# zhenfeizhang/falcon-r1cs

Measured on AMD Instinct MI355X. Metric: falcon1024_verify_with_ntt_r1cs_witnesses_per_sec, higher is better.
Workload: dtype u32; 1 GPU; falcon-1024 full verify-with-ntt witness (NTT ladder + mod_q + pointwise + l2-norm), batch=65536 signatures per GPU per step (BASELINE configs[2] on every GPU); logn=10, batch_per_gpu=65536, chunk=32768, encoding=bls12-381-fr montgomery (arkworks witness_assignment bytes), seed=0x46414c434f4e31, signatures_failing_range_checks=0, ranks_seen=1, hbm_plan_bytes=166888865792, hbm_plan_limit_bytes=259200000000

## Files before the change

### falcon-r1cs_amd/csrc/frw_prepare.hip

```cpp
#include <hip/hip_runtime.h>
#include <stdint.h>
#include <algorithm>
#include "frw_device.h"
#include "frw_keccak.h"
#include "frw_layout.h"

namespace frw {

constexpr int SHAKE256_RATE = 136;
constexpr int NONCE_LEN = 40;

__device__ __forceinline__ void hash_to_point_one(int logn, const uint8_t *__restrict__ nonce, const uint8_t *__restrict__ msg, uint64_t o0,
                                         uint64_t o1, uint16_t *__restrict__ out)
{
    const int n = 1 << logn;
    const size_t total = NONCE_LEN + (size_t)(o1 >= o0 ? o1 - o0 : 0);
    uint64_t st[25];
#pragma unroll
    for (int i = 0; i < 25; i++) st[i] = 0;
    for (size_t pos = 0;; pos += SHAKE256_RATE) {
#pragma unroll
        for (int l = 0; l < SHAKE256_RATE / 8; l++) {
            uint64_t w = 0;
#pragma unroll
            for (int b = 0; b < 8; b++) {
                const size_t p = pos + (size_t)(l * 8 + b);
                uint32_t byte = 0;
                if (p < NONCE_LEN) byte = nonce[p];
                else if (p < total) byte = msg[p - NONCE_LEN];
                else if (p == total) byte = 0x1F;
                w |= (uint64_t)byte << (8 * b);
            }
            st[l] ^= w;
        }
        const bool last = total < pos + SHAKE256_RATE;
        if (last) st[16] ^= 0x8000000000000000ull;
        keccak_f1600(st);
        if (last) break;
    }
    int cnt = 0;
    while (cnt < n) {
#pragma unroll
        for (int w = 0; w < SHAKE256_RATE / 2; w++) {
            const uint64_t lane = st[w / 4];
            const int sh = (w % 4) * 16;
            const uint32_t v = (uint32_t)((lane >> sh) & 0xff) << 8 | (uint32_t)((lane >> (sh + 8)) & 0xff);
            if (v < 5 * Q && cnt < n) out[cnt++] = (uint16_t)(v % Q);
        }
        if (cnt < n) keccak_f1600(st);
    }
}

__global__ __launch_bounds__(BLOCK) void hash_to_point_kernel(int logn, size_t batch, const uint8_t *__restrict__ nonces,
                                                              const uint8_t *__restrict__ msgs,
                                                              const uint64_t *__restrict__ msg_off, uint16_t *__restrict__ hm)
{
    const size_t s = (size_t)blockIdx.x * blockDim.x + threadIdx.x;
    if (s >= batch) return;
    const uint64_t o0 = msg_off[s], o1 = msg_off[s + 1];
    hash_to_point_one(logn, nonces + s * NONCE_LEN, msgs + o0, o0, o1, hm + (s << logn));
}

__device__ __forceinline__ uint32_t public_key_coeff(const uint8_t *__restrict__ p, int k)
{
    const int bit = 14 * k, off = bit & 7;
    const uint8_t *q = p + 1 + (bit >> 3);
    uint32_t acc = (uint32_t)q[0] << 16 | (uint32_t)q[1] << 8;
    if (off + 14 > 16) acc |= q[2];
    return (acc >> (24 - 14 - off)) & 0x3fffu;
}

__global__ __launch_bounds__(BLOCK) void decode_public_keys_kernel(int logn, size_t batch, const uint8_t *__restrict__ pk_bytes,
                                                                   uint16_t *__restrict__ pk, int32_t *__restrict__ status)
{
    const int n = 1 << logn;
    const size_t pk_len = 1 + (size_t)14 * n / 8;
    const size_t idx = (size_t)blockIdx.x * blockDim.x + threadIdx.x;
    if (idx >= batch * (size_t)n) return;
    const size_t s = idx >> logn;
    const int k = (int)(idx & (size_t)(n - 1));
    const uint8_t *p = pk_bytes + s * pk_len;
    const uint32_t c = public_key_coeff(p, k);
    pk[idx] = (uint16_t)c;
    if (c >= Q || (k == 0 && p[0] != (uint8_t)logn)) atomicMax(&status[s], ST_DECODE);
}

__device__ __forceinline__ bool decode_signature_one(int logn, const uint8_t *__restrict__ p, size_t sig_len, uint16_t *__restrict__ out,
                                            uint8_t *__restrict__ nonce_out)
{
    const int n = 1 << logn;
    bool ok = sig_len > 1 + NONCE_LEN && p[0] == (uint8_t)(0x30 + logn);
    if (ok && nonce_out)
        for (int i = 0; i < NONCE_LEN; i++) nonce_out[i] = p[1 + i];
    const uint8_t *body = p + 1 + NONCE_LEN;
    const size_t body_len = ok ? sig_len - 1 - NONCE_LEN : 0;
    size_t v = 0;
    uint32_t acc = 0;
    int acc_len = 0;
    for (int u = 0; ok && u < n; u++) {
        if (v >= body_len) { ok = false; break; }
        acc = (acc << 8) | body[v++];
        const uint32_t b = acc >> acc_len;
        const uint32_t sign = b & 128u;
        uint32_t m = b & 127u;
        for (;;) {
            if (acc_len == 0) {
                if (v >= body_len) { ok = false; break; }
                acc = (acc << 8) | body[v++];
                acc_len = 8;
            }
            acc_len--;
            if ((acc >> acc_len) & 1u) break;
            m += 128;
            if (m > 2047) { ok = false; break; }
        }
        if (sign && m == 0) ok = false;
        if (ok) out[u] = (uint16_t)(sign ? Q - m : m);
    }
    if (ok && (acc & ((1u << acc_len) - 1u))) ok = false;
    for (; ok && v < body_len; v++)
        if (body[v]) ok = false;
    return ok;
}

__global__ __launch_bounds__(BLOCK) void decode_signatures_kernel(int logn, size_t batch, const uint8_t *__restrict__ sig_bytes,
                                                                  size_t sig_len, uint16_t *__restrict__ sig,
                                                                  uint8_t *__restrict__ nonce_out, int32_t *__restrict__ status)
{
    const size_t s = (size_t)blockIdx.x * blockDim.x + threadIdx.x;
    if (s >= batch) return;
    const bool ok = decode_signature_one(logn, sig_bytes + s * sig_len, sig_len, sig + (s << logn),
                                         nonce_out ? nonce_out + s * NONCE_LEN : nullptr);
    status[s] = ok ? ST_OK : ST_DECODE;
}

__global__ __launch_bounds__(BLOCK) void agg_hash_to_point_kernel(int logn, size_t count, const uint32_t *__restrict__ stmt,
                                                                  const uint8_t *__restrict__ nonces, const uint8_t *__restrict__ msgs,
                                                                  const uint64_t *__restrict__ msg_off, uint16_t *__restrict__ hm)
{
    const size_t k = (size_t)blockIdx.x * blockDim.x + threadIdx.x;
    if (k >= count) return;
    const size_t s = stmt[k];
    const uint64_t o0 = msg_off[s], o1 = msg_off[s + 1];
    hash_to_point_one(logn, nonces + aggregate_route(logn - 9, k, s).nonce_off, msgs + o0, o0, o1, hm + (k << logn));
}

__global__ __launch_bounds__(BLOCK) void agg_decode_public_keys_kernel(int logn, size_t count, const uint32_t *__restrict__ stmt,
                                                                       const uint8_t *__restrict__ pk_bytes, uint16_t *__restrict__ pk,
                                                                       int32_t *__restrict__ status)
{
    const int n = 1 << logn;
    const size_t idx = (size_t)blockIdx.x * blockDim.x + threadIdx.x;
    if (idx >= count * (size_t)n) return;
    const size_t k = idx >> logn;
    const int j = (int)(idx & (size_t)(n - 1));
    const uint8_t *p = pk_bytes + aggregate_route(logn - 9, k, stmt[k]).pk_off;
    const uint32_t c = public_key_coeff(p, j);
    pk[idx] = (uint16_t)c;
    if (c >= Q || (j == 0 && p[0] != (uint8_t)logn)) atomicMax(&status[k], ST_DECODE);
}

__global__ __launch_bounds__(BLOCK) void agg_decode_signatures_kernel(int logn, size_t count, const uint32_t *__restrict__ stmt,
                                                                      const uint8_t *__restrict__ sig_bytes, uint16_t *__restrict__ sig,
                                                                      uint8_t *__restrict__ nonces, int32_t *__restrict__ status)
{
    const size_t k = (size_t)blockIdx.x * blockDim.x + threadIdx.x;
    if (k >= count) return;
    const AggRoute r = aggregate_route(logn - 9, k, stmt[k]);
    const uint8_t *p = sig_bytes + r.sig_off;
    for (int i = 0; i < NONCE_LEN; i++) nonces[r.nonce_off + i] = p[1 + i];
    status[k] = decode_signature_one(logn, p, aggregate_sig_len(logn - 9), sig + (k << logn), nullptr) ? ST_OK : ST_DECODE;
}

struct AggVerdicts { const uint32_t *stmt[2]; const int32_t *status[2]; const uint64_t *norm[2]; uint32_t count[2]; };
__global__ __launch_bounds__(BLOCK) void agg_scatter_verdicts_kernel(AggVerdicts v, int32_t *__restrict__ status, uint64_t *__restrict__ norm)
{
    size_t k = (size_t)blockIdx.x * blockDim.x + threadIdx.x;
    int g = 0;
    if (k >= v.count[0]) { k -= v.count[0]; g = 1; }
    if (k >= v.count[g]) return;
    const size_t s = v.stmt[g][k];
    status[s] = v.status[g][k];
    if (norm) norm[s] = v.norm[g][k];
}

__global__ __launch_bounds__(BLOCK) void agg_count_refused_kernel(size_t count, const int32_t *__restrict__ status, uint32_t *__restrict__ refused)
{
    __shared__ uint32_t wave_count[WAVES];
    uint32_t mine = 0;
    for (size_t s = threadIdx.x; s < count; s += BLOCK) mine += status[s] != ST_OK;
#pragma unroll
    for (int off = WAVE / 2; off > 0; off >>= 1) mine += __shfl_xor(mine, off, WAVE);
    if ((threadIdx.x & (WAVE - 1)) == 0) wave_count[threadIdx.x / WAVE] = mine;
    __syncthreads();
    if (threadIdx.x == 0) {
        uint32_t total = 0;
#pragma unroll
        for (int w = 0; w < WAVES; w++) total += wave_count[w];
        refused[0] = total;
    }
}


__device__ inline uint32_t pok_block_rank(bool flag, uint32_t &total)
{
    __shared__ uint32_t wave_count[WAVES];
    const uint64_t mask = __ballot(flag);
    const int lane = threadIdx.x & (WAVE - 1), wave = threadIdx.x / WAVE;
    if (lane == 0) wave_count[wave] = (uint32_t)__popcll(mask);
    __syncthreads();
    uint32_t before = 0;
    total = 0;
#pragma unroll
    for (int w = 0; w < WAVES; w++) {
        if (w < wave) before += wave_count[w];
        total += wave_count[w];
    }
    return before + (uint32_t)__popcll(mask & (((uint64_t)1 << lane) - 1));
}

__global__ __launch_bounds__(BLOCK) void pok_scan_count_kernel(size_t batch, const int32_t *__restrict__ status,
                                                               uint32_t *__restrict__ block_sums)
{
    const size_t s = (size_t)blockIdx.x * BLOCK + threadIdx.x;
    uint32_t total;
    (void)pok_block_rank(s < batch && status[s] == ST_OK, total);
    if (threadIdx.x == 0) block_sums[blockIdx.x] = total;
}

__global__ __launch_bounds__(BLOCK) void pok_scan_offsets_kernel(size_t num_blocks, uint32_t *__restrict__ block_sums,
                                                                 uint32_t *__restrict__ count)
{
    __shared__ uint32_t wave_sum[WAVES];
    const int lane = threadIdx.x & (WAVE - 1), wave = threadIdx.x / WAVE;
    uint32_t carry = 0;
    for (size_t base = 0; base < num_blocks; base += BLOCK) {
        const size_t i = base + threadIdx.x;
        const uint32_t v = i < num_blocks ? block_sums[i] : 0;
        uint32_t incl = v;
#pragma unroll
        for (int d = 1; d < WAVE; d <<= 1) {
            const uint32_t up = __shfl_up(incl, d, WAVE);
            if (lane >= d) incl += up;
        }
        if (lane == WAVE - 1) wave_sum[wave] = incl;
        __syncthreads();
        uint32_t before = 0, tile = 0;
#pragma unroll
        for (int w = 0; w < WAVES; w++) {
            if (w < wave) before += wave_sum[w];
            tile += wave_sum[w];
        }
        if (i < num_blocks) block_sums[i] = carry + before + incl - v;
        carry += tile;
        __syncthreads();
    }
    if (threadIdx.x == 0) count[0] = carry;
}

__global__ __launch_bounds__(BLOCK) void pok_scan_write_kernel(size_t batch, const int32_t *__restrict__ status,
                                                               const uint32_t *__restrict__ block_offsets, uint32_t *__restrict__ index)
{
    const size_t s = (size_t)blockIdx.x * BLOCK + threadIdx.x;
    const bool ok = s < batch && status[s] == ST_OK;
    uint32_t total;
    const uint32_t rank = pok_block_rank(ok, total);
    if (ok) index[block_offsets[blockIdx.x] + rank] = (uint32_t)s;
}

__global__ __launch_bounds__(BLOCK) void pok_gather_rs_kernel(size_t count, const uint32_t *__restrict__ index,
                                                              const uint64_t *__restrict__ rs, uint64_t *__restrict__ dense_rs)
{
    const size_t t = (size_t)blockIdx.x * BLOCK + threadIdx.x;
    if (t >= count * 8) return;
    dense_rs[t] = rs[(size_t)index[t / 8] * 8 + (t & 7)];
}

__global__ __launch_bounds__(BLOCK) void pok_gather_inputs_kernel(int logn, const uint32_t *__restrict__ index,
                                                                  const uint16_t *__restrict__ sig, const uint16_t *__restrict__ pk,
                                                                  const uint16_t *__restrict__ hm, uint16_t *__restrict__ sig_out,
                                                                  uint16_t *__restrict__ pk_out, uint16_t *__restrict__ hm_out)
{
    const size_t j = blockIdx.x, slot = index[j];
    const uint32_t row = (2u << logn) / 16;
    for (uint32_t t = threadIdx.x; t < 3 * row; t += BLOCK) {
        const uint32_t a = t / row, v = t % row;
        const uint16_t *src = a == 0 ? sig : a == 1 ? pk : hm;
        uint16_t *dst = a == 0 ? sig_out : a == 1 ? pk_out : hm_out;
        ((uint4 *)dst)[j * row + v] = ((const uint4 *)src)[slot * row + v];
    }
}

struct PokOutputs { uint8_t *wire; uint64_t *proofs, *instance; uint32_t *unsatisfied; uint32_t wire_len, inst_words; };

__global__ __launch_bounds__(BLOCK) void pok_zero_refused_kernel(size_t batch, const int32_t *__restrict__ status, PokOutputs out)
{
    for (size_t s = blockIdx.x; s < batch; s += gridDim.x) {
        if (status[s] == ST_OK) continue;
        for (uint32_t t = threadIdx.x; t < out.wire_len; t += BLOCK) out.wire[s * out.wire_len + t] = 0;
        if (out.proofs && threadIdx.x < 48) out.proofs[s * 48 + threadIdx.x] = 0;
        if (out.instance)
            for (uint32_t t = threadIdx.x; t < out.inst_words; t += BLOCK) out.instance[s * out.inst_words + t] = 0;
        if (out.unsatisfied && threadIdx.x == 0) out.unsatisfied[s] = 0;
    }
}

__global__ __launch_bounds__(BLOCK) void pok_scatter_kernel(const uint32_t *__restrict__ index, const uint8_t *__restrict__ wire,
                                                            const uint64_t *__restrict__ proofs, const uint64_t *__restrict__ instance,
                                                            const uint32_t *__restrict__ unsatisfied, PokOutputs out)
{
    const size_t j = blockIdx.x, s = index[j];
    for (uint32_t t = threadIdx.x; t < out.wire_len; t += BLOCK) out.wire[s * out.wire_len + t] = wire[j * out.wire_len + t];
    if (out.proofs && threadIdx.x < 48) out.proofs[s * 48 + threadIdx.x] = proofs[j * 48 + threadIdx.x];
    if (out.instance)
        for (uint32_t t = threadIdx.x; t < out.inst_words; t += BLOCK) out.instance[s * out.inst_words + t] = instance[j * out.inst_words + t];
    if (out.unsatisfied && threadIdx.x == 0) out.unsatisfied[s] = unsatisfied[j];
}

hipError_t launch_pok_scan(size_t batch, const int32_t *status, uint32_t *block_sums, uint32_t *index, uint32_t *count, hipStream_t st)
{
    if (batch == 0) return hipSuccess;
    const size_t blocks = (batch + BLOCK - 1) / BLOCK;
    hipLaunchKernelGGL(pok_scan_count_kernel, dim3((unsigned)blocks), dim3(BLOCK), 0, st, batch, status, block_sums);
    hipLaunchKernelGGL(pok_scan_offsets_kernel, dim3(1), dim3(BLOCK), 0, st, blocks, block_sums, count);
    hipLaunchKernelGGL(pok_scan_write_kernel, dim3((unsigned)blocks), dim3(BLOCK), 0, st, batch, status, (const uint32_t *)block_sums, index);
    return hipGetLastError();
}

hipError_t launch_pok_gather_rs(size_t count, const uint32_t *index, const uint64_t *rs, uint64_t *dense_rs, hipStream_t st)
{
    if (count == 0) return hipSuccess;
    hipLaunchKernelGGL(pok_gather_rs_kernel, dim3((unsigned)((count * 8 + BLOCK - 1) / BLOCK)), dim3(BLOCK), 0, st, count, index, rs, dense_rs);
    return hipGetLastError();
}

hipError_t launch_pok_gather_inputs(int logn, size_t cnt, const uint32_t *index, const uint16_t *sig, const uint16_t *pk, const uint16_t *hm,
                                    uint16_t *sig_out, uint16_t *pk_out, uint16_t *hm_out, hipStream_t st)
{
    if (cnt == 0) return hipSuccess;
    hipLaunchKernelGGL(pok_gather_inputs_kernel, dim3((unsigned)cnt), dim3(BLOCK), 0, st, logn, index, sig, pk, hm, sig_out, pk_out, hm_out);
    return hipGetLastError();
}

hipError_t launch_pok_zero_refused(size_t batch, const int32_t *status, int wire_len, int inst_words, uint8_t *wire, uint64_t *proofs,
                                   uint64_t *instance, uint32_t *unsatisfied, hipStream_t st)
{
    if (batch == 0) return hipSuccess;
    const PokOutputs out = {wire, proofs, instance, unsatisfied, (uint32_t)wire_len, (uint32_t)inst_words};
    hipLaunchKernelGGL(pok_zero_refused_kernel, dim3((unsigned)std::min<size_t>(batch, 65536)), dim3(BLOCK), 0, st, batch, status, out);
    return hipGetLastError();
}

hipError_t launch_pok_scatter(size_t cnt, const uint32_t *index, int wire_len, int inst_words, const uint8_t *wire_in,
                              const uint64_t *proofs_in, const uint64_t *instance_in, const uint32_t *unsatisfied_in, uint8_t *wire,
                              uint64_t *proofs, uint64_t *instance, uint32_t *unsatisfied, hipStream_t st)
{
    if (cnt == 0) return hipSuccess;
    const PokOutputs out = {wire, proofs, instance, unsatisfied, (uint32_t)wire_len, (uint32_t)inst_words};
    hipLaunchKernelGGL(pok_scatter_kernel, dim3((unsigned)cnt), dim3(BLOCK), 0, st, index, wire_in, proofs_in, instance_in, unsatisfied_in, out);
    return hipGetLastError();
}

hipError_t launch_hash_to_point(int logn, size_t batch, const uint8_t *nonces, const uint8_t *msgs, const uint64_t *msg_off,
                                uint16_t *hm, hipStream_t st)
{
    if (batch == 0) return hipSuccess;
    hipLaunchKernelGGL(hash_to_point_kernel, dim3((unsigned)((batch + BLOCK - 1) / BLOCK)), dim3(BLOCK), 0, st, logn, batch, nonces,
                       msgs, msg_off, hm);
    return hipGetLastError();
}

hipError_t launch_decode_public_keys(int logn, size_t batch, const uint8_t *pk_bytes, uint16_t *pk, int32_t *status, hipStream_t st)
{
    if (batch == 0) return hipSuccess;
    hipError_t e = hipMemsetAsync(status, 0, batch * sizeof(int32_t), st);
    if (e != hipSuccess) return e;
    const size_t total = batch << logn;
    hipLaunchKernelGGL(decode_public_keys_kernel, dim3((unsigned)((total + BLOCK - 1) / BLOCK)), dim3(BLOCK), 0, st, logn, batch,
                       pk_bytes, pk, status);
    return hipGetLastError();
}

hipError_t launch_decode_signatures(int logn, size_t batch, const uint8_t *sig_bytes, size_t sig_len, uint16_t *sig,
                                    uint8_t *nonce_out, int32_t *status, hipStream_t st)
{
    if (batch == 0) return hipSuccess;
    hipLaunchKernelGGL(decode_signatures_kernel, dim3((unsigned)((batch + BLOCK - 1) / BLOCK)), dim3(BLOCK), 0, st, logn, batch,
                       sig_bytes, sig_len, sig, nonce_out, status);
    return hipGetLastError();
}

hipError_t launch_agg_hash_to_point(int logn, size_t count, const uint32_t *stmt, const uint8_t *nonces, const uint8_t *msgs,
                                    const uint64_t *msg_off, uint16_t *hm, hipStream_t st)
{
    if (count == 0) return hipSuccess;
    hipLaunchKernelGGL(agg_hash_to_point_kernel, dim3((unsigned)((count + BLOCK - 1) / BLOCK)), dim3(BLOCK), 0, st, logn, count, stmt, nonces,
                       msgs, msg_off, hm);
    return hipGetLastError();
}

hipError_t launch_agg_decode_public_keys(int logn, size_t count, const uint32_t *stmt, const uint8_t *pk_bytes, uint16_t *pk, int32_t *status,
                                         hipStream_t st)
{
    if (count == 0) return hipSuccess;
    hipError_t e = hipMemsetAsync(status, 0, count * sizeof(int32_t), st);
    if (e != hipSuccess) return e;
    const size_t total = count << logn;
    hipLaunchKernelGGL(agg_decode_public_keys_kernel, dim3((unsigned)((total + BLOCK - 1) / BLOCK)), dim3(BLOCK), 0, st, logn, count, stmt,
                       pk_bytes, pk, status);
    return hipGetLastError();
}

hipError_t launch_agg_decode_signatures(int logn, size_t count, const uint32_t *stmt, const uint8_t *sig_bytes, uint16_t *sig, uint8_t *nonces,
                                        int32_t *status, hipStream_t st)
{
    if (count == 0) return hipSuccess;
    hipLaunchKernelGGL(agg_decode_signatures_kernel, dim3((unsigned)((count + BLOCK - 1) / BLOCK)), dim3(BLOCK), 0, st, logn, count, stmt,
                       sig_bytes, sig, nonces, status);
    return hipGetLastError();
}

hipError_t launch_agg_verdicts(const uint32_t *const stmt[2], const int32_t *const set_status[2], const uint64_t *const set_norm[2],
                               const size_t count[2], int32_t *status, uint64_t *norm, uint32_t *refused, hipStream_t st)
{
    const size_t total = count[0] + count[1];
    if (total == 0) return hipSuccess;
    const AggVerdicts v = {{stmt[0], stmt[1]}, {set_status[0], set_status[1]}, {set_norm[0], set_norm[1]}, {(uint32_t)count[0], (uint32_t)count[1]}};
    hipLaunchKernelGGL(agg_scatter_verdicts_kernel, dim3((unsigned)((total + BLOCK - 1) / BLOCK)), dim3(BLOCK), 0, st, v, status, norm);
    hipLaunchKernelGGL(agg_count_refused_kernel, dim3(1), dim3(BLOCK), 0, st, total, (const int32_t *)status, refused);
    return hipGetLastError();
}

}
```

Before: 1.341 million signatures/s.

## Decode signatures with 16-byte vector loads and a branchless bit-stream decoder

Replaces the byte-at-a-time Falcon signature decoder with a streaming decoder that fetches 16-byte granules with prefetch-ahead, decodes coefficients via count-leading-zeros on a 64-bit bit buffer, and writes eight packed coefficients per 16-byte store. The decode kernel now launches one wave per block, and the public-key decode error flag uses a wave ballot so only one lane issues the atomic. The aim is to cut the per-byte load and store traffic and the branchy per-bit loop in the per-signature serial decode. It adds a bytewise fallback path and relies on aligned output and a correct reimplementation of the validity checks.

```diff
diff --git a/falcon-r1cs_amd/csrc/frw_prepare.hip b/falcon-r1cs_amd/csrc/frw_prepare.hip
--- a/falcon-r1cs_amd/csrc/frw_prepare.hip
+++ b/falcon-r1cs_amd/csrc/frw_prepare.hip
@@ -4,11 +4,13 @@
 #include "frw_device.h"
 #include "frw_keccak.h"
 #include "frw_layout.h"
+#include "frw_sigdecode.h"
 
 namespace frw {
 
 constexpr int SHAKE256_RATE = 136;
 constexpr int NONCE_LEN = 40;
+static_assert(SIG_Q == Q && SIG_NONCE_LEN == NONCE_LEN, "frw_sigdecode.h is the same codec");
 
 __device__ __forceinline__ void hash_to_point_one(int logn, const uint8_t *__restrict__ nonce, const uint8_t *__restrict__ msg, uint64_t o0,
                                          uint64_t o1, uint16_t *__restrict__ out)
@@ -82,50 +84,28 @@
     const uint8_t *p = pk_bytes + s * pk_len;
     const uint32_t c = public_key_coeff(p, k);
     pk[idx] = (uint16_t)c;
-    if (c >= Q || (k == 0 && p[0] != (uint8_t)logn)) atomicMax(&status[s], ST_DECODE);
-}
-
-__device__ __forceinline__ bool decode_signature_one(int logn, const uint8_t *__restrict__ p, size_t sig_len, uint16_t *__restrict__ out,
-                                            uint8_t *__restrict__ nonce_out)
-{
-    const int n = 1 << logn;
-    bool ok = sig_len > 1 + NONCE_LEN && p[0] == (uint8_t)(0x30 + logn);
-    if (ok && nonce_out)
-        for (int i = 0; i < NONCE_LEN; i++) nonce_out[i] = p[1 + i];
-    const uint8_t *body = p + 1 + NONCE_LEN;
-    const size_t body_len = ok ? sig_len - 1 - NONCE_LEN : 0;
-    size_t v = 0;
-    uint32_t acc = 0;
-    int acc_len = 0;
-    for (int u = 0; ok && u < n; u++) {
-        if (v >= body_len) { ok = false; break; }
-        acc = (acc << 8) | body[v++];
-        const uint32_t b = acc >> acc_len;
-        const uint32_t sign = b & 128u;
-        uint32_t m = b & 127u;
-        for (;;) {
-            if (acc_len == 0) {
-                if (v >= body_len) { ok = false; break; }
-                acc = (acc << 8) | body[v++];
-                acc_len = 8;
-            }
-            acc_len--;
-            if ((acc >> acc_len) & 1u) break;
-            m += 128;
-            if (m > 2047) { ok = false; break; }
-        }
-        if (sign && m == 0) ok = false;
-        if (ok) out[u] = (uint16_t)(sign ? Q - m : m);
-    }
-    if (ok && (acc & ((1u << acc_len) - 1u))) ok = false;
-    for (; ok && v < body_len; v++)
-        if (body[v]) ok = false;
-    return ok;
-}
-
-__global__ __launch_bounds__(BLOCK) void decode_signatures_kernel(int logn, size_t batch, const uint8_t *__restrict__ sig_bytes,
-                                                                  size_t sig_len, uint16_t *__restrict__ sig,
-                                                                  uint8_t *__restrict__ nonce_out, int32_t *__restrict__ status)
+    const bool bad = c >= Q || (k == 0 && p[0] != (uint8_t)logn);
+    if (__ballot(bad) != 0 && (threadIdx.x & (WAVE - 1)) == 0) atomicMax(&status[s], ST_DECODE);
+}
+
+__global__ __launch_bounds__(WAVE) void decode_signatures_kernel(int logn, size_t batch, const uint8_t *__restrict__ sig_bytes,
+                                                                 size_t sig_len, uint16_t *__restrict__ sig,
+                                                                 uint8_t *__restrict__ nonce_out, int32_t *__restrict__ status)
+{
+    const size_t s = (size_t)blockIdx.x * blockDim.x + threadIdx.x;
+    if (s >= batch) return;
+    const uint8_t *p = sig_bytes + s * sig_len;
+    const uint32_t lead = (uint32_t)((uintptr_t)p & 15);
+    const uint4 *span = (const uint4 *)(p - lead);
+    uint4 *row = (uint4 *)(sig + (s << logn));
+    const bool ok = decode_signature_wide(logn, p, lead, sig_len, nonce_out ? nonce_out + s * NONCE_LEN : nullptr,
+                                          [span](uint32_t g) { return span[g]; }, [row](uint32_t j, const uint4 &v) { row[j] = v; });
+    status[s] = ok ? ST_OK : ST_DECODE;
+}
+
+__global__ __launch_bounds__(BLOCK) void decode_signatures_bytewise_kernel(int logn, size_t batch, const uint8_t *__restrict__ sig_bytes,
+                                                                           size_t sig_len, uint16_t *__restrict__ sig,
+                                                                           uint8_t *__restrict__ nonce_out, int32_t *__restrict__ status)
 {
     const size_t s = (size_t)blockIdx.x * blockDim.x + threadIdx.x;
     if (s >= batch) return;
@@ -385,8 +365,12 @@
                                     uint8_t *nonce_out, int32_t *status, hipStream_t st)
 {
     if (batch == 0) return hipSuccess;
-    hipLaunchKernelGGL(decode_signatures_kernel, dim3((unsigned)((batch + BLOCK - 1) / BLOCK)), dim3(BLOCK), 0, st, logn, batch,
-                       sig_bytes, sig_len, sig, nonce_out, status);
+    if (((uintptr_t)sig & 15) == 0 && sig_len > 1 + NONCE_LEN && sig_len < SIG_WIDE_MAX_LEN)
+        hipLaunchKernelGGL(decode_signatures_kernel, dim3((unsigned)((batch + WAVE - 1) / WAVE)), dim3(WAVE), 0, st, logn, batch, sig_bytes,
+                           sig_len, sig, nonce_out, status);
+    else
+        hipLaunchKernelGGL(decode_signatures_bytewise_kernel, dim3((unsigned)((batch + BLOCK - 1) / BLOCK)), dim3(BLOCK), 0, st, logn, batch,
+                           sig_bytes, sig_len, sig, nonce_out, status);
     return hipGetLastError();
 }
 
diff --git a/falcon-r1cs_amd/csrc/frw_sigdecode.h b/falcon-r1cs_amd/csrc/frw_sigdecode.h
--- /dev/null
+++ b/falcon-r1cs_amd/csrc/frw_sigdecode.h
@@ -0,0 +1,150 @@
+#pragma once
+#include <hip/hip_runtime.h>
+#include <stddef.h>
+#include <stdint.h>
+
+namespace frw {
+
+constexpr uint32_t SIG_Q = 12289;
+constexpr int SIG_NONCE_LEN = 40;
+constexpr size_t SIG_WIDE_MAX_LEN = (size_t)1 << 28;
+
+__host__ __device__ __forceinline__ bool decode_signature_one(int logn, const uint8_t *__restrict__ p, size_t sig_len, uint16_t *__restrict__ out,
+                                                     uint8_t *__restrict__ nonce_out)
+{
+    const int n = 1 << logn;
+    bool ok = sig_len > 1 + SIG_NONCE_LEN && p[0] == (uint8_t)(0x30 + logn);
+    if (ok && nonce_out)
+        for (int i = 0; i < SIG_NONCE_LEN; i++) nonce_out[i] = p[1 + i];
+    const uint8_t *body = p + 1 + SIG_NONCE_LEN;
+    const size_t body_len = ok ? sig_len - 1 - SIG_NONCE_LEN : 0;
+    size_t v = 0;
+    uint32_t acc = 0;
+    int acc_len = 0;
+    for (int u = 0; ok && u < n; u++) {
+        if (v >= body_len) { ok = false; break; }
+        acc = (acc << 8) | body[v++];
+        const uint32_t b = acc >> acc_len;
+        const uint32_t sign = b & 128u;
+        uint32_t m = b & 127u;
+        for (;;) {
+            if (acc_len == 0) {
+                if (v >= body_len) { ok = false; break; }
+                acc = (acc << 8) | body[v++];
+                acc_len = 8;
+            }
+            acc_len--;
+            if ((acc >> acc_len) & 1u) break;
+            m += 128;
+            if (m > 2047) { ok = false; break; }
+        }
+        if (sign && m == 0) ok = false;
+        if (ok) out[u] = (uint16_t)(sign ? SIG_Q - m : m);
+    }
+    if (ok && (acc & ((1u << acc_len) - 1u))) ok = false;
+    for (; ok && v < body_len; v++)
+        if (body[v]) ok = false;
+    return ok;
+}
+
+template <class Store>
+struct SigStream {
+    uint64_t buf;
+    int valid;
+    uint32_t skip, rem, u, n, tail, min_unary, max_coeff, o0, o1, o2, o3;
+    Store store;
+
+    __host__ __device__ __forceinline__ SigStream(int logn, uint32_t lead, size_t sig_len, Store store_)
+        : buf(0), valid(0), skip(8 * (lead + 1 + SIG_NONCE_LEN)), rem(8 * (uint32_t)(sig_len - 1 - SIG_NONCE_LEN)), u(0), n(1u << logn), tail(0),
+          min_unary(0xffffffffu), max_coeff(0), o0(0), o1(0), o2(0), o3(0), store(store_) {}
+
+    __host__ __device__ __forceinline__ bool refused() const { return min_unary < 0x10000u || max_coeff >= SIG_Q; }
+
+    __host__ __device__ __forceinline__ void drain()
+    {
+        while (valid >= 24 && u < n) {
+            const uint32_t hi = (uint32_t)(buf >> 32);
+            const uint32_t unary = hi << 8;
+            const uint32_t k = unary ? (uint32_t)__builtin_clz(unary) : 32u;
+            const uint32_t m = ((hi >> 24) & 127u) | (k << 7);
+            const uint32_t c = (int32_t)hi < 0 ? SIG_Q - m : m;
+            min_unary = unary < min_unary ? unary : min_unary;
+            max_coeff = c > max_coeff ? c : max_coeff;
+            buf <<= 9 + k;
+            valid -= 9 + (int)k;
+            o0 = (o0 >> 16) | (o1 << 16);
+            o1 = (o1 >> 16) | (o2 << 16);
+            o2 = (o2 >> 16) | (o3 << 16);
+            o3 = (o3 >> 16) | (c << 16);
+            if ((u & 7) == 7) store(u >> 3, make_uint4(o0, o1, o2, o3));
+            u++;
+        }
+        const bool done = u == n;
+        tail |= done ? (uint32_t)(buf != 0) : 0u;
+        buf = done ? 0 : buf;
+        valid = done ? 0 : valid;
+    }
+
+    __host__ __device__ __forceinline__ void word(uint32_t le)
+    {
+        const uint32_t drop = skip < 32 ? skip : 32, bits = 32 - drop, take = bits < rem ? bits : rem;
+        uint32_t w = drop < 32 ? __builtin_bswap32(le) << drop : 0u;
+        w = take ? w & (0xffffffffu << (32 - take)) : 0u;
+        skip -= drop;
+        rem -= take;
+        const bool done = u == n;
+        tail |= done ? w : 0u;
+        buf |= (uint64_t)(done ? 0u : w) << (32 - valid);
+        valid += done ? 0 : (int)bits;
+        drain();
+    }
+
+    __host__ __device__ __forceinline__ bool granule(const uint4 &q)
+    {
+        word(q.x);
+        word(q.y);
+        word(q.z);
+        word(q.w);
+        return !refused();
+    }
+
+    __host__ __device__ __forceinline__ bool finish()
+    {
+        while (u < n) {
+            valid += 32;
+            drain();
+            if (refused()) return false;
+        }
+        return tail == 0;
+    }
+};
+
+template <class Fetch, class Store>
+__host__ __device__ __forceinline__ bool decode_signature_wide(int logn, const uint8_t *__restrict__ p, uint32_t lead, size_t sig_len,
+                                                      uint8_t *__restrict__ nonce_out, Fetch fetch, Store store)
+{
+    const uint32_t last = (uint32_t)((lead + sig_len - 1) >> 4);
+    if (p[0] != (uint8_t)(0x30 + logn)) return false;
+    if (nonce_out)
+        for (int i = 0; i < SIG_NONCE_LEN; i++) nonce_out[i] = p[1 + i];
+    const auto ahead = [&](uint32_t g) { return fetch(g < last ? g : last); };
+    uint4 q0 = ahead(0), q1 = ahead(1), q2 = ahead(2), q3 = ahead(3);
+    SigStream<Store> s(logn, lead, sig_len, store);
+    for (uint32_t g = 0;; g += 4) {
+        if (!s.granule(q0)) return false;
+        q0 = ahead(g + 4);
+        if (g + 1 > last) break;
+        if (!s.granule(q1)) return false;
+        q1 = ahead(g + 5);
+        if (g + 2 > last) break;
+        if (!s.granule(q2)) return false;
+        q2 = ahead(g + 6);
+        if (g + 3 > last) break;
+        if (!s.granule(q3)) return false;
+        q3 = ahead(g + 7);
+        if (g + 4 > last) break;
+    }
+    return s.finish();
+}
+
+}
```

Result: no change. 1.347 million signatures/s, median of 3 (+0.4%).
